# skim0119/gym-softrobot

Hardware: AMD Instinct MI355X
Metric: env_steps_per_sec (higher is better)
Workload: dtype f64

## Files before the change

gym_softrobot_amd/_capi.py:

```python
from __future__ import annotations

import ctypes as C
import os
from pathlib import Path

ABI_VERSION = 17

FEAT_GRAVITY = 1 << 0
FEAT_POINT_FORCE_NODE0_X = 1 << 1
FEAT_PENDULUM_BC = 1 << 2
FEAT_ANALYTICAL_DAMPER = 1 << 3
FEAT_FIXED_BC = 1 << 4
FEAT_TIP_FORCE = 1 << 5
FEAT_MOVING_BASE_BC = 1 << 6
FEAT_LAPLACE_FILTER = 1 << 7
FEAT_PLANE_CONTACT_ANISO = 1 << 8
FEAT_REST_KAPPA_ACTION = 1 << 9
FEAT_OCTO_HEAD = 1 << 10
FEAT_SPLINE_MUSCLE_TORQUES = 1 << 11
FEAT_SUCKER_CONSTRAINT = 1 << 12
FEAT_COOMM_MUSCLES = 1 << 13
MAX_SUCKERS = 4
MAX_MUSCLES = 4
MUSCLE_LONGITUDINAL = 0
# ... 957 lines not shown
    "softrod_bank_info": (C.c_int, [_VP, C.POINTER(C.c_int32), C.POINTER(C.c_uint64), _VP]),
    "softrod_camera_default": (C.c_int, [C.POINTER(SoftrodConfig), C.POINTER(SoftrodCamera)]),
    "softrod_camera_check": (C.c_int, [C.POINTER(SoftrodCamera)]),
    "softrod_render": (C.c_int, [_VP, C.POINTER(SoftrodCamera), _VP, _VP, _VP]),
    "softrod_rod_clearance": (C.c_int, [_VP, C.c_int, _VP, _VP]),
    "softrod_set_rod_shape": (C.c_int, [_VP, _VP, _VP, _VP, _VP, _VP, _VP]),
    "softrod_set_reset_shapes": (C.c_int, [_VP, C.c_int, _VP, _VP, _VP, _VP, C.c_uint64, _VP]),
    "softrod_apply_reset_shapes": (C.c_int, [_VP, _VP, _VP]),
    "softrod_reset_shapes_view": (C.c_int, [_VP, C.POINTER(C.c_void_p), C.POINTER(C.c_void_p)]),
    "softrod_reset_shape_index": (C.c_uint32, [C.c_uint64, C.c_uint32, C.c_uint32, C.c_uint32]),
    "softrod_substeps": (C.c_int, [_VP, _VP, C.c_int, _VP]),
    "softrod_state_view_get": (C.c_int, [_VP, C.POINTER(SoftrodStateView)]),
    "softrod_set_timing": (C.c_int, [_VP, C.c_int]),
    "softrod_kernel_times_ms": (C.c_int, [_VP, _VP, C.c_int, C.POINTER(C.c_int)]),
    "softrod_last_kernel_ms": (C.c_int, [_VP, C.POINTER(C.c_float)]),
    "softrod_kernel_tier": (C.c_char_p, [_VP]),
    "softrod_last_error": (C.c_char_p, [_VP]),
    "softrod_destroy": (C.c_int, [_VP]),
}

EXPORTED_SYMBOLS = tuple(_EXPORTS)

_lib = None


def library_path() -> Path:
    env = os.environ.get("SOFTROD_HIP_LIB")
    if env:
        return Path(env)
    return Path(__file__).resolve().parent / "csrc" / "libsoftrod_hip.so"
# ... 52 lines not shown
```

gym_softrobot_amd/backend.py:

```python
from __future__ import annotations

import ctypes as C
from typing import Dict, Optional, Tuple

import numpy as np
import torch

from . import _capi
from ._capi import LANE_STRIDE, SoftrodConfig, SoftrodStateView, check, load_library
from .diagnostics import (JointLoads, MuscleLoads, RodClearance, RodDynamics, RodStrains, joint_loads_views,
                          muscle_loads_views, rod_clearance_views, rod_dynamics_views, rod_strains_views)


class _DevArray:

    def __init__(self, ptr: int, shape, typestr: str, owner):
        self._owner = owner
        self.__cuda_array_interface__ = {
            "shape": tuple(shape),
            "typestr": typestr,
            "data": (int(ptr), False),
            "version": 2,
            "strides": None,
        }
# ... 478 lines not shown
    def set_timing(self, n_launches: int) -> None:
        check(self._lib.softrod_set_timing(self._h, int(n_launches)), self._h)

    def kernel_times_ms(self) -> np.ndarray:
        cap = 1 << 16
        out = np.zeros(cap, np.float32)
        cnt = C.c_int()
        check(self._lib.softrod_kernel_times_ms(self._h, out.ctypes.data, cap, C.byref(cnt)), self._h)
        return out[: cnt.value].copy()

    def last_kernel_ms(self) -> float:
        ms = C.c_float()
        check(self._lib.softrod_last_kernel_ms(self._h, C.byref(ms)), self._h)
        return float(ms.value)

    def prev_action_rows(self) -> torch.Tensor:
        if getattr(self, "_prev_rows", None) is None:
            self._prev_rows = self.state()["prev_action"]
            if not self.is_octo and not self.is_mocto:
                self._prev_rows = self._prev_rows[:, : self.action_dim]
        return self._prev_rows

    def state(self) -> Dict[str, torch.Tensor]:
        v = SoftrodStateView()
        check(self._lib.softrod_state_view_get(self._h, C.byref(v)), self._h)
        n, s = self.n_envs, int(v.lane_stride)

        def view(ptr, comps):
            return torch.as_tensor(_DevArray(ptr, (comps, n, s), "<f8", self), device=self.device)

# ... 152 lines not shown
```

gym_softrobot_amd/csrc/softrod_capi.hip:

```cpp
#include <hip/hip_runtime.h>
#include <hip/hip_ext.h>

#include <cmath>
#include <cstdio>
#include <cstdlib>
#include <cstring>
#include <new>
#include <string>
#include <vector>

#include "softrod_kernels.hpp"
#include "softrod_dynamics_readout.hpp"
#include "softrod_copy_envs.hpp"
#include "softrod_state_bank.hpp"
#include "softrod_shape.hpp"
#include "softrod_reset_shapes.hpp"

using namespace softrod;

template <class Row>
struct EnvTable {
    Row* dev = nullptr;
    Row* host = nullptr;
    hipEvent_t ev = nullptr;
// ... 48 lines not shown
    RodParams* d_params = nullptr;
    StatePtrs* d_state = nullptr;
    double* d_time_tab = nullptr;
    double* d_mat = nullptr;
    double* d_render_radius = nullptr;
    double* d_mtab = nullptr;
    bool muscles_set = false;
    unsigned* d_ticket = nullptr;
    bool tapered = false;
    bool was_reset = false;
    bool basis_set = false;
    double* h_init = nullptr;
    uint8_t* h_mask = nullptr;
    std::vector<hipEvent_t> ev_start, ev_stop;
    int timed = 0;
    hipEvent_t ev_reset = nullptr;
    int q_depth = 0;
    double* d_queue = nullptr;
    double* h_queue = nullptr;
    int* d_consumed = nullptr;
    int* d_produced = nullptr;
    int* d_underflow = nullptr;
    uint8_t* d_flags = nullptr;
    int* h_produced = nullptr;
    std::vector<int> seen_consumed;
    std::vector<int2> pending;
    double* h_stage = nullptr;
    int2* h_where = nullptr;
    double* d_stage = nullptr;
    int2* d_where = nullptr;
// ... 233 lines not shown
    return SOFTROD_OK;
}

int launch_autoreset_same_step(softrod_handle* h, float* obs, double* aux, int pack, hipStream_t st) {
    const dim3 grid((unsigned)h->cfg.n_envs), block(kLanes * h->nw);
    if (restarts_as_body(h))
        hipLaunchKernelGGL(softrod_octo_autoreset_same_step_kernel, grid, block, 0, st, h->P, h->S, obs, pack, h->d_final_obs,
                           h->d_final_time);
    else
        hipLaunchKernelGGL(by_epl(h, softrod_autoreset_same_step_kernel<1>, softrod_autoreset_same_step_kernel<2>), grid, block,
                           0, st, h->P, h->S, obs, aux, pack, h->d_final_obs, h->d_final_time, h->d_final_aux);
    SR_HIP(h, hipGetLastError());
    return SOFTROD_OK;
}

int launch_reset_shapes(softrod_handle* h, int mode, const uint8_t* mask, float* obs, const uint8_t* term, const uint8_t* trunc,
                        double* aux, int pack, hipStream_t st) {
    const int N = h->cfg.n_envs;
    ResetShapesPick pick{};
    pick.index = h->d_rs_index; pick.episode = h->d_rs_episode; pick.picked = h->d_rs_picked;
    pick.seed = h->rs_seed; pick.count = h->rs_count; pick.mode = mode; pick.mask = mask;
    pick.terminated = pack ? nullptr : term; pick.truncated = pack ? nullptr : trunc;
    pick.packed = (mode == kPickFinished && pack) ? obs : nullptr;
    pick.od = softrod_config_obs_dim(&h->cfg);
    hipLaunchKernelGGL(softrod_reset_shapes_pick_kernel, dim3((unsigned)((N + kPickThreads - 1) / kPickThreads)), dim3(kPickThreads),
                       0, st, h->P, h->S, pick);
    const RodLayout y = rod_layout(h);
    const RodShapeArgs args{h->d_rs_field[0], h->d_rs_field[1], h->d_rs_field[2], h->d_rs_field[3], h->d_rs_picked, h->d_rs_index};
    hipLaunchKernelGGL(by_epl(h, softrod_rod_shape_kernel<1>, softrod_rod_shape_kernel<2>), dim3((unsigned)(N * y.rods)),
                       dim3(kLanes), 0, st, h->P, h->S, y.rods, y.lane_stride, y.arm_stride, args);
// ... 3 lines not shown
                               h->d_rs_picked, obs, pack);
        else
            hipLaunchKernelGGL(by_epl(h, softrod_observe_kernel<1>, softrod_observe_kernel<2>), dim3((unsigned)N), dim3(kLanes), 0,
                               st, h->P, h->S, h->d_rs_picked, nullptr, obs, aux, pack);
    }
    SR_HIP(h, hipGetLastError());
    return SOFTROD_OK;
}

enum : unsigned { kOptMuscles = SOFTROD_FEAT_COOMM_MUSCLES, kOptEarlyTerm = kFeatEarlyTerm, kOptEnvMaterial = kFeatEnvMaterial,
                  kOptEnvContact = kFeatEnvContact, kOptCompiledFor = kOptEarlyTerm | kOptEnvMaterial | kOptEnvContact };
constexpr int kAny = -1, kMoctoEnvs = -2;
constexpr unsigned kAnyFeatures = kRuntimeFeatures;
using StepKernel = void (*)(RodParams, StatePtrs, const float*, float*, double*, uint8_t*, uint8_t*, double*, int, int, int);
using OctoKernel = void (*)(RodParams, StatePtrs, const float*, float*, double*, uint8_t*, uint8_t*, int, int, int);
using WindowKernel = void (*)(RodParams, StatePtrs, const float*, int, int);

struct StepRow {
    unsigned feats;
    int env;
    int math, epl;
    int taper, zup;
    int nw_min, nw_max;
    bool windowed;
    unsigned needs, honours;
    StepKernel step; OctoKernel octo; WindowKernel window;
    int epb, waves;
    const char* label;
};

constexpr StepRow compiled_row(unsigned F, int env, int epl, int taper, int nw_min, int nw_max, const char* label) {
// ... 198 lines not shown
        if (!mask || mask[i]) build(values + W * i, T.host[i]);
    SR_HIP(h, hipMemcpyAsync(T.dev, T.host, N * sizeof(Row), hipMemcpyHostToDevice, st));
    SR_HIP(h, hipEventRecord(T.ev, st));
    return SOFTROD_OK;
}

template <class K, class... A>
void launch_stamped(K kernel, const dim3& grid, const dim3& block, hipStream_t st, hipEvent_t t0, hipEvent_t t1, A... args) {
    if (t0 || t1) hipExtLaunchKernelGGL(kernel, grid, block, 0, st, t0, t1, 0, args...);
    else hipLaunchKernelGGL(kernel, grid, block, 0, st, args...);
}

int launch_step(softrod_handle* h, const float* actions, float* obs, double* reward,
                uint8_t* term, uint8_t* trunc, double* aux, int n_sub, int epilogue, int pack,
                hipStream_t st) {
    if (h->q_depth > 0 && epilogue && !h->same_step) {
        if (const int rc = launch_autoreset(h, obs, reward, term, trunc, aux, pack, st)) return rc;
        if (h->rs_count > 0)
            if (const int rc = launch_reset_shapes(h, kPickSkipped, nullptr, obs, term, trunc, aux, pack, st)) return rc;
    }
    if ((h->cfg.features & SOFTROD_FEAT_COOMM_MUSCLES) && h->cfg.math_mode == SOFTROD_MATH_FAST) {
        const bool push = h->cfg.env_kind == SOFTROD_ENV_ARM_PUSH || is_pull(h) || is_mocto(h);
        if (is_mocto(h) && (!h->tapered || !h->muscles_set || (h->cfg.env_kind == SOFTROD_ENV_ARM_TWO && !h->basis_set)))
            return fail(h, SOFTROD_EINVAL, "the muscle octopus needs softrod_set_radius_profile and softrod_set_muscle_layers "
                                           "(and SOFTROD_ENV_ARM_TWO softrod_set_action_basis) before it steps");
        if (push && !h->tapered)
            return fail(h, SOFTROD_EINVAL, "SOFTROD_ENV_ARM_PUSH (SOFTROD_MATH_FAST): call softrod_set_radius_profile first "
                                           "(the reference's arm is tapered, arm_push_env.py:160-179)");
        if (!push && h->tapered)
            return fail(h, SOFTROD_EINVAL, "a tapered muscle rod outside SOFTROD_ENV_ARM_PUSH runs under SOFTROD_MATH_LIBM only");
    }
    const StepChoice c = select_step(h, epilogue);
    if (!c.row) return fail(h, SOFTROD_EINVAL, c.why);
    const StepChoice after = c.row->windowed ? select_step(h, 0) : StepChoice{nullptr, nullptr};
    if (c.row->windowed && !after.row) return fail(h, SOFTROD_EINVAL, after.why);
    auto launch = [&](const StepRow& r, int n, int epi, hipEvent_t t0, hipEvent_t t1) {
        const dim3 grid((unsigned)((h->cfg.n_envs + r.epb - 1) / r.epb)), block(kLanes * (r.waves ? r.waves : h->nw));
        if (r.window) launch_stamped(r.window, grid, block, st, t0, t1, h->P, h->S, actions, n, h->window_refresh);
        else if (r.octo) launch_stamped(r.octo, grid, block, st, t0, t1, h->P, h->S, actions, obs, reward, term, trunc, n, epi, pack);
        else launch_stamped(r.step, grid, block, st, t0, t1, h->P, h->S, actions, obs, reward, term, trunc, aux, n, epi, pack);
    };
    const bool timing = h->timed < (int)h->ev_start.size();
    const hipEvent_t t0 = timing ? h->ev_start[h->timed] : nullptr, t1 = timing ? h->ev_stop[h->timed] : nullptr;
    const bool mocto = c.row->env == kMoctoEnvs;
    const bool action_first = mocto && epilogue && actions, epilogue_last = mocto && epilogue;
    const dim3 grid((unsigned)h->cfg.n_envs), block(kLanes * h->nw);
    if (action_first)
        launch_stamped(softrod_mocto_action_kernel, grid, block, st, t0, nullptr, h->P, h->S, actions, n_sub);
    launch(*c.row, n_sub, epilogue, action_first ? nullptr : t0, (after.row || epilogue_last) ? nullptr : t1);
    if (after.row) launch(*after.row, 0, 1, nullptr, epilogue_last ? nullptr : t1);
    if (epilogue_last)
        launch_stamped(softrod_mocto_epilogue_kernel, grid, block, st, nullptr, t1, h->P, h->S, obs, reward, term, trunc, 1, pack);
    SR_HIP(h, hipGetLastError());
    if (timing) ++h->timed;
    if (h->q_depth > 0 && epilogue && h->same_step) {
        if (const int rc = launch_autoreset_same_step(h, obs, aux, pack, st)) return rc;
        if (h->rs_count > 0)
            if (const int rc = launch_reset_shapes(h, kPickFinished, nullptr, obs, term, trunc, aux, pack, st)) return rc;
    }
    return SOFTROD_OK;
}

int upload_and_reset(softrod_handle* h, hipStream_t st, bool use_mask) {
    const size_t N = (size_t)h->cfg.n_envs;
    SR_HIP(h, hipMemcpyAsync(h->d_init, h->h_init, N * h->init_stride * sizeof(double), hipMemcpyHostToDevice, st));
    if (use_mask)
        SR_HIP(h, hipMemcpyAsync(h->d_mask, h->h_mask, N, hipMemcpyHostToDevice, st));
    ResetArgs A{h->d_init, use_mask ? h->d_mask : nullptr};
    if (is_octo(h)) {
        OctoResetArgs OA{h->d_init, h->d_init + N * (size_t)h->cfg.n_arm * 18, use_mask ? h->d_mask : nullptr};
        hipLaunchKernelGGL(softrod_octo_reset_kernel, dim3((unsigned)N), dim3(kLanes * h->nw), 0, st, h->P, h->S, OA);
    } else
        hipLaunchKernelGGL(by_epl(h, softrod_reset_kernel<1>, softrod_reset_kernel<2>), dim3((unsigned)N), dim3(kLanes), 0, st,
// ... 1227 lines not shown
        return fail(h, SOFTROD_EINVAL, "null argument");
    if (const int rc = step_preconditions(h)) return rc;
    SR_ON_DEVICE(h);
    return launch_step(h, actions, obs, reward, terminated, truncated, aux, h->cfg.n_substeps, 1, 0,
                       (hipStream_t)stream);
}

int softrod_step_packed(softrod_handle* h, const float* actions, float* packed, double* aux, void* stream) {
    if (!h || !actions || !packed) return fail(h, SOFTROD_EINVAL, "null argument");
    if (const int rc = step_preconditions(h)) return rc;
    SR_ON_DEVICE(h);
    return launch_step(h, actions, packed, nullptr, nullptr, nullptr, aux, h->cfg.n_substeps, 1, 1,
                       (hipStream_t)stream);
}

namespace {
struct PeerTable { float* p[SOFTROD_MAX_PEERS]; };
__global__ void __launch_bounds__(256) softrod_scatter_rows_kernel(const float* __restrict__ packed, PeerTable peers,
                                                                   int n_peers, size_t n_words, size_t offset,
                                                                   long long tag_word, unsigned tag,
                                                                   unsigned* __restrict__ ticket) {
    const size_t i = (size_t)blockIdx.x * blockDim.x + threadIdx.x;
    if (i < n_words) {
        const float v = packed[i];
        for (int q = 0; q < n_peers; ++q)
            __hip_atomic_store(&peers.p[q][offset + i], v, __ATOMIC_RELAXED, __HIP_MEMORY_SCOPE_SYSTEM);
    }
    if (tag_word < 0) return;
    asm volatile("s_waitcnt vmcnt(0)" ::: "memory");
    __syncthreads();
// ... 591 lines not shown
```

gym_softrobot_amd/csrc/softrod_fast.hpp:

```cpp
#pragma once

namespace softrod {

__device__ __forceinline__ bool wave_any(bool p) { return __builtin_amdgcn_ballot_w64(p) != 0ull; }
__device__ __forceinline__ bool wave_any_of(unsigned long long lanes, bool p) {
    return (__builtin_amdgcn_ballot_w64(p) & lanes) != 0ull;
}

__device__ __forceinline__ double horner(double g, double y, double c) {
    double d;
    asm("v_fma_f64 %0, %1, %2, %3" : "=v"(d) : "v"(g), "v"(y), "v"(c));
    return d;
}
__device__ __forceinline__ void fma_over(double& d, double a, double b, double c) {
    asm("v_fma_f64 %0, %1, %2, %3" : "+v"(d) : "v"(a), "v"(b), "v"(c));
}
__device__ __forceinline__ void fma_inplace_u(double& x, double m, double a) {
    asm("v_fma_f64 %0, %1, %0, %2" : "+v"(x) : "s"(m), "v"(a));
}

template <bool LEAN = true, bool ON_CIRCLE = false>
__device__ __forceinline__ void sinc_cosc(double t, double& sc, double& cc) {
    if (!wave_any(t >= 1.0e-3)) {
        if constexpr (LEAN) {
// ... 467 lines not shown
#if SOFTROD_IDLE_LANES_EXEC_MASK
    if (has<F>(P, SOFTROD_FEAT_SPLINE_MUSCLE_TORQUES) || slot_local<F>(P, lane * EPL) <= P.n_elem)
#endif
    {
        constexpr bool kOnCircle = F == kRuntimeFeatures || (F & ~kFeatEnvMaterial) != SOFTROD_FEATURES_SOFTPENDULUM;
        kinematic_n<EPL, kOnCircle>(P.half_dt, C, L);
        ProgressPriority prio(n_sub);
        for (int s = 0; s < n_sub; ++s) {
            dynamic_n<F, EPL, TAPER>(Pk, C, B, lane, L);
            const bool last = (s == n_sub - 1);
            kinematic_n<EPL, kOnCircle>(last ? P.half_dt : P.dt, C, L);
            prio.tick(s);
        }
    }
}
template <unsigned F, int E, int EPL>
__device__ __attribute__((noinline)) void general_step_cold(const RodParams* __restrict__ params,
                                                            const StatePtrs* __restrict__ sp, int rod, int lane,
                                                            const float* __restrict__ actions, int n_sub, int poison) {
    const RodParams P = *params;
    const StatePtrs S = *sp;
    const size_t N = (size_t)P.n_envs;
    LaneN<EPL> L;
    double time;
    if (poison) {
        poison_rod<EPL>(L);
        time = S.time[rod];
    } else {
        load_lane<EPL, F>(S, N, rod, lane, L);
        BcTargets B;
        load_bc(S, N, rod, B);
        EnvAction A;
        set_action_n<F, E, EPL>(P, S, N, rod, lane, actions, A, B, L);
        constrain_rates_n<F, EPL>(P, B, lane, L);
        constrain_values_n<F, EPL>(P, B, lane, L);
        time = S.time[rod];
        if (n_sub > 0) {
            ConstN<EPL> C;
            if constexpr (kEnvMaterial<F>) build_const_m<F, EPL>(P, S.env_mat[rod], lane, A, C);
            else build_const<F, EPL>(P, lane, A, C);
// ... 30 lines not shown
#else
#define SR_PHASE(i) do {} while (0)
#endif

template <unsigned F, int EPL, bool TAPER>
constexpr int fast_kernel_waves() {
    if (EPL > 1) return 1;
    if (F == kRuntimeFeatures) return SOFTROD_RUNTIME_WAVES;
    if (F & (SOFTROD_FEAT_PLANE_CONTACT_ANISO | SOFTROD_FEAT_LAPLACE_FILTER | SOFTROD_FEAT_SPLINE_MUSCLE_TORQUES |
             SOFTROD_FEAT_COOMM_MUSCLES))
        return SOFTROD_CONTACT_WAVES;
    if (TAPER) return SOFTROD_CONTACT_WAVES;
    return (F & ~kFeatEnvMaterial) == SOFTROD_FEATURES_SOFTPENDULUM ? SOFTROD_PLANAR_WAVES : SOFTROD_FAST_WAVES;
}

template <unsigned F, int E, int EPL, bool TAPER = false>
__global__ void __launch_bounds__(kLanes, (fast_kernel_waves<F, EPL, TAPER>()))
softrod_step_fast_kernel(const RodParams P, const StatePtrs S, const float* __restrict__ actions,
                         float* __restrict__ obs, double* __restrict__ reward,
                         uint8_t* __restrict__ terminated, uint8_t* __restrict__ truncated,
                         double* __restrict__ aux, const int n_sub, const int epilogue, const int pack) {
    const int rod = blockIdx.x;
    const int lane = threadIdx.x;
    const size_t N = (size_t)P.n_envs;
    [[maybe_unused]] EnvMaterial M;
    if constexpr (kEnvMaterial<F>) M = S.env_mat[rod];
    [[maybe_unused]] EnvContact CT;
    if constexpr (kEnvContact<F>) CT = S.env_contact[rod];
    if (epilogue && S.skip && S.skip[rod]) {
        if (lane == 0) S.skip[rod] = 0;
        if (lane == 0 && early_term_on<F>(P)) S.aux[rod] = 0.0;
        return;
    }

    __builtin_amdgcn_s_setprio(3);
    SR_PHASE(0);
    constexpr bool kPlanarKernel = (F & ~kFeatEnvMaterial) == SOFTROD_FEATURES_SOFTPENDULUM;
    LaneN<EPL> L;
    load_lane<EPL, F, !kPlanarKernel>(S, N, rod, lane, L);
    SR_PHASE(1);
    if (has<F>(P, SOFTROD_FEAT_LAPLACE_FILTER)) sanitize_unused_rates<EPL>(P, lane, L);
    if (has<F>(P, SOFTROD_FEAT_PLANE_CONTACT_ANISO)) sanitize_unused_slots<EPL>(P, lane, L);
    BcTargets B;
    load_bc(S, N, rod, B);
    load_suckers<F>(P, S, N, rod, B);
    EnvAction A;
    set_action_n<F, E, EPL>(P, S, N, rod, lane, actions, A, B, L);
    if (epilogue) push_store_prev_com<F, E, EPL>(P, S, N, rod, lane, L, n_sub);
    if (has<F>(P, SOFTROD_FEAT_SPLINE_MUSCLE_TORQUES)) muscle_load<EPL>(P, S, rod, actions != nullptr, A, L);
    {
        BcTargets B0 = B;
        if (has<F>(P, SOFTROD_FEAT_MOVING_BASE_BC)) {
            B0.vel[0] = __shfl(L.v[0][0], 0); B0.vel[1] = __shfl(L.v[0][1], 0); B0.vel[2] = __shfl(L.v[0][2], 0);
        }
        constrain_rates_n<F, EPL>(P, B0, lane, L);
        constrain_values_n<F, EPL>(P, B, lane, L);
    }
    double time = S.time[rod];
    ConstN<EPL> C;
    if constexpr (kEnvMaterial<F>) build_const_m<F, EPL, TAPER>(P, M, lane, A, C, S.mat);
    else build_const_m<F, EPL, TAPER>(P, P, lane, A, C, S.mat);
    if constexpr (kEnvContact<F>) C.ct = CT;
    if constexpr (kMusclesCompiled<F>) build_muscle_const<F, EPL, true>(P, S, N, rod, lane, A, C);
    RodParams Pk = P;
    if (!has<F>(P, SOFTROD_FEAT_ANALYTICAL_DAMPER)) Pk.damp_t = 1.0;

    bool blown_up = false;
    if (n_sub > 0 && epilogue && rod_has_nan<EPL>(P, lane, L)) {
        blown_up = true;
        if constexpr (!kPlanarKernel) {
            poison_rod<EPL>(L);
            time = clock_after(P, S, time, n_sub);
        }
    }
    if constexpr (kPlanarKernel) {
        PlanarN<EPL> Z;
        if (n_sub > 0 && !blown_up && planar_from_lane<EPL>(P, B, lane, L, Z)) {
            PlanarC<EPL> K;
            planar_build_const<EPL, kEnvMaterial<F>>(Pk, C, lane, K);
            const double ta = P.time_two_half_adds ? P.half_dt : P.dt;
            const double tb = P.time_two_half_adds ? P.half_dt : 0.0;
            int tk = -1;
            if (S.time_tab && n_sub == P.tab_n_sub) {
                const double kf = rint(time * P.inv_step_time);
                const int k = (kf >= 0.0 && kf < (double)(P.tab_len - 1)) ? (int)kf : -1;
                tk = (k >= 0 && S.time_tab[k] == time) ? k : -1;
            }
            const double step_dt = EPL > 1 ? opaque_v(P.dt) : P.dt;
            SR_PHASE(2);
#if SOFTROD_PLANAR_EXEC_MASK
            if (lane * EPL <= P.n_elem) {
#endif
// ... 24 lines not shown
#endif
            if (__builtin_amdgcn_readfirstlane(tk) >= 0) time = S.time_tab[tk + 1];
            else
                for (int s = 0; s < n_sub; ++s) time = (time + ta) + tb;
            SR_PHASE(3);
            planar_store<EPL>(S, N, rod, lane, Z, !SOFTROD_PLANAR_EXEC_MASK || lane * EPL <= P.n_elem);
#pragma unroll
            for (int s = 0; s < EPL; ++s) {
#pragma unroll
                for (int c = 0; c < 3; ++c) { L.x[s][c] = 0.0; L.v[s][c] = 0.0; L.w[s][c] = 0.0; L.t[s][c] = 0.0; }
#pragma unroll
                for (int c = 0; c < 9; ++c) L.Q[s][c] = 0.0;
            }
            planar_to_lane<EPL>(Z, L);
        } else {
            general_step_cold<F, E, EPL>(S.params, S.self, rod, lane, actions, n_sub, blown_up);
            __builtin_amdgcn_fence(__ATOMIC_ACQUIRE, "wavefront");
            load_lane<EPL, F>(S, N, rod, opaque_lane(lane), L);
            time = S.time[rod];
        }
    } else {
        if (n_sub > 0 && !blown_up) {
            general_substeps<F, EPL, TAPER>(P, Pk, C, B, lane, L, n_sub);
            time = clock_after(P, S, time, n_sub);
        }
        store_lane<EPL, F>(S, N, rod, lane, L);
    }
    if (has<F>(P, SOFTROD_FEAT_SPLINE_MUSCLE_TORQUES)) muscle_store<EPL>(P, S, rod, lane, L);
    if (env_of<E>(P) == SOFTROD_ENV_SOFT_ARM && lane == 0)
        S.ctrl[(size_t)0 * N + rod] += (double)n_sub;
    if (lane == 0) S.time[rod] = time;
// ... 9 lines not shown
```

gym_softrobot_amd/csrc/softrod_kernels.hpp:

```cpp
#pragma once
#include <hip/hip_runtime.h>
#include <stdint.h>

#include "../../include/softrod.h"

namespace softrod {

constexpr int kLanes = 64;

constexpr unsigned kRuntimeFeatures = 0xFFFFFFFFu;
constexpr unsigned kFeaturesTaperedSuckerArm = SOFTROD_FEAT_ANALYTICAL_DAMPER | SOFTROD_FEAT_SUCKER_CONSTRAINT;
constexpr unsigned kFeatPlaneZup = 1u << 30;
constexpr unsigned kFeatEarlyTerm = 1u << 29;
constexpr unsigned kFeatEnvMaterial = 1u << 28;
template <unsigned F>
constexpr bool kEnvMaterial = F != kRuntimeFeatures && (F & kFeatEnvMaterial) != 0;
constexpr unsigned kFeatEnvContact = 1u << 27;
template <unsigned F>
constexpr bool kEnvContact = F != kRuntimeFeatures && (F & kFeatEnvContact) != 0;
constexpr int kRuntimeEnv = -1;
constexpr unsigned kFeaturesMuscleRod = SOFTROD_FEAT_FIXED_BC | SOFTROD_FEAT_ANALYTICAL_DAMPER | SOFTROD_FEAT_COOMM_MUSCLES;
template <unsigned F>
constexpr bool kMusclesCompiled = F != kRuntimeFeatures && (F & SOFTROD_FEAT_COOMM_MUSCLES) != 0;

// ... 1587 lines not shown
        sucker_rates_n<kRuntimeFeatures, 1>(P, B, lane, L);
    }
    if (P.features & SOFTROD_FEAT_ANALYTICAL_DAMPER) {
        L.v[0][0] *= M.damp_t; L.v[0][1] *= M.damp_t; L.v[0][2] *= M.damp_t;
        L.w[0][0] *= pow(M.damp_r[0], e);
        L.w[0][1] *= pow(M.damp_r[1], e);
        L.w[0][2] *= pow(M.damp_r[2], e);
    }
    if (P.features & SOFTROD_FEAT_LAPLACE_FILTER) laplace_filter_rates_n<1>(P, lane, L);
    if (P.damp_before_constrain) {
        constrain_rates_n<kRuntimeFeatures, 1>(P, B, lane, L);
        sucker_rates_n<kRuntimeFeatures, 1>(P, B, lane, L);
    }
}

#ifndef SOFTROD_LIBM_WAVES
#define SOFTROD_LIBM_WAVES 1
#endif
template <bool ET>
__global__ void __launch_bounds__(kLanes, SOFTROD_LIBM_WAVES)
softrod_step_libm_kernel(const RodParams P, const StatePtrs S, const float* __restrict__ actions,
                         float* __restrict__ obs, double* __restrict__ reward,
                         uint8_t* __restrict__ terminated, uint8_t* __restrict__ truncated,
                         double* __restrict__ aux, const int n_sub, const int epilogue, const int pack) {
    const int rod = blockIdx.x;
    const int lane = threadIdx.x;
    const size_t N = (size_t)P.n_envs;
    if (epilogue && S.skip && S.skip[rod]) {
        if (lane == 0) S.skip[rod] = 0;
        if (ET && lane == 0) S.aux[rod] = 0.0;
        return;
    }

    LaneN<1> L;
    load_lane<1, kRuntimeFeatures>(S, N, rod, lane, L);
    BcTargets B;
    load_bc(S, N, rod, B);
    load_suckers<kRuntimeFeatures>(P, S, N, rod, B);
    EnvAction A;
    set_action_n<kRuntimeFeatures, kRuntimeEnv, 1>(P, S, N, rod, lane, actions, A, B, L);
    if (epilogue) push_store_prev_com<kRuntimeFeatures, kRuntimeEnv, 1>(P, S, N, rod, lane, L, n_sub);
    ConstN<1> C;
    const EnvMaterial E = env_material_rt(P, S, rod);
// ... 60 lines not shown
        double a[EPL], o[EPL];
#pragma unroll
        for (int s = 0; s < EPL; ++s) a[s] = x[s][c];
        shift_next<EPL>(a, o);
#pragma unroll
        for (int s = 0; s < EPL; ++s) t[s][c] = o[s] - x[s][c];
    }
#pragma unroll
    for (int s = 0; s < EPL; ++s) {
        const double len = sqrt(t[s][0] * t[s][0] + t[s][1] * t[s][1] + t[s][2] * t[s][2]) + P.eps_length;
#pragma unroll
        for (int c = 0; c < 3; ++c) t[s][c] /= len;
    }
}

__device__ __forceinline__ const double* staged_record(const StatePtrs& S, size_t N, int env, int k) {
    if (k >= S.q_produced[env]) {
        if (threadIdx.x == 0) atomicAdd(S.q_underflow, 1);
        return nullptr;
    }
    return S.queue + ((size_t)(k % S.q_depth) * N + env) * (size_t)S.q_record;
}

template <int EPL>
__global__ void __launch_bounds__(kLanes)
softrod_observe_kernel(const RodParams P, const StatePtrs S, const uint8_t* __restrict__ picked,
                       const float* __restrict__ prev_action, float* __restrict__ obs, double* __restrict__ aux,
                       const int pack) {
    const int rod = blockIdx.x;
    if (picked && !picked[rod]) return;
    const int lane = threadIdx.x;
    const size_t N = (size_t)P.n_envs;
    LaneN<EPL> L;
    load_lane<EPL, kRuntimeFeatures>(S, N, rod, lane, L);
    const int adim = (P.env_kind == SOFTROD_ENV_SOFTPENDULUM3D) ? 2
                   : (P.env_kind == SOFTROD_ENV_ARM_SINGLE) ? 7 : (P.env_kind == SOFTROD_ENV_SOFT_ARM) ? 0
// ... 77 lines not shown
    LaneN<EPL> L;
    reset_rod<EPL>(P, S, (size_t)P.n_envs, rod, threadIdx.x, A.init + (size_t)rod * 18, L);
}

__global__ void __launch_bounds__(kLanes)
softrod_queue_scatter_kernel(double* __restrict__ queue, const double* __restrict__ staged,
                             const int2* __restrict__ where, const int n_envs, const int record) {
    const int m = blockIdx.x;
    const int2 w = where[m];
    double* dst = queue + ((size_t)w.y * (size_t)n_envs + (size_t)w.x) * (size_t)record;
    const double* src = staged + (size_t)m * (size_t)record;
    for (int i = threadIdx.x; i < record; i += kLanes) dst[i] = src[i];
}

template <int EPL>
__global__ void __launch_bounds__(kLanes)
softrod_autoreset_kernel(const RodParams P, const StatePtrs S, float* __restrict__ obs,
                         double* __restrict__ reward, uint8_t* __restrict__ terminated,
                         uint8_t* __restrict__ truncated, double* __restrict__ aux, const int pack) {
    const int rod = blockIdx.x;
    const int lane = threadIdx.x;
    if (!S.needs_reset[rod]) return;
    const size_t N = (size_t)P.n_envs;
    const int k = S.q_consumed[rod];
    const double* in = staged_record(S, N, rod, k);
    if (!in) return;
    LaneN<EPL> L;
    reset_rod<EPL>(P, S, N, rod, lane, in, L);
    float pa[7];
#pragma unroll
    for (int i = 0; i < 7; ++i) pa[i] = S.prev_action[7 * (size_t)rod + i];
    float* o = observe_rod<EPL>(P, S, N, rod, lane, L, pa, obs, pack, aux);
    if (lane == 0) {
        emit_scalars(o, env_obs_dim(P), pack, rod, 0.0, false, false, reward, terminated, truncated, S.needs_reset);
        S.skip[rod] = 1;
        S.q_consumed[rod] = k + 1;
    }
}

}

#include "softrod_fast.hpp"
#include "softrod_octo.hpp"
#include "softrod_window.hpp"
#include "softrod_literal.hpp"
#include "softrod_readout.hpp"
#include "softrod_reaction.hpp"
#include "softrod_strains.hpp"
#include "softrod_muscle_readout.hpp"
#include "softrod_joint_readout.hpp"
#include "softrod_render.hpp"
#include "softrod_clearance.hpp"
// ... 2 lines not shown
```

gym_softrobot_amd/csrc/softrod_window.hpp:

```cpp
#pragma once

namespace softrod {

constexpr int kWindowRho = 4;

template <unsigned F>
__device__ __forceinline__ void window_load(const StatePtrs& S, size_t N, int rod, int g, LaneN<1>& L) {
    constexpr size_t W = 2 * kLanes;
    const size_t m = (size_t)rod * W + (size_t)g;
#pragma unroll
    for (int c = 0; c < 3; ++c) {
        L.x[0][c] = S.pos[c * N * W + m];
        L.v[0][c] = S.vel[c * N * W + m];
        L.w[0][c] = S.omg[c * N * W + m];
        L.t[0][c] = S.tan[c * N * W + m];
        L.kap[0][c] = S.kap[c * N * W + m];
        L.rk[0][c] = S.rkap[c * N * W + m];
    }
#pragma unroll
    for (int c = 0; c < 9; ++c) L.Q[0][c] = S.dir[c * N * W + m];
}

__device__ __forceinline__ void window_store(const StatePtrs& S, size_t N, int rod, int g, const LaneN<1>& L) {
    constexpr size_t W = 2 * kLanes;
// ... 1 lines not shown
#pragma unroll
    for (int c = 0; c < 3; ++c) {
        S.pos[c * N * W + m] = L.x[0][c];
        S.vel[c * N * W + m] = L.v[0][c];
        S.omg[c * N * W + m] = L.w[0][c];
        S.tan[c * N * W + m] = L.t[0][c];
        S.kap[c * N * W + m] = L.kap[0][c];
    }
#pragma unroll
    for (int c = 0; c < 9; ++c) S.dir[c * N * W + m] = L.Q[0][c];
}

template <unsigned F, int RPB = 1>
__global__ void __launch_bounds__(2 * kLanes * RPB, SOFTROD_CONTACT_WAVES)
softrod_step_window_kernel(const RodParams P, const StatePtrs S, const float* __restrict__ actions,
                           const int n_sub, const int refresh) {
    static_assert(RPB == 1 || RPB == 4, "one rod per workgroup, or four with partner waves on one SIMD");
    constexpr int kFields = 18;
    constexpr int kHalo = (RPB == 1) ? kLanes : 32;
    constexpr int kBuf = (RPB == 1) ? 1 : 2;
    __shared__ double ex_[RPB][kBuf][2][kFields][kHalo];
    __shared__ int flag_[RPB][2];
    __shared__ int sany_[RPB];

    const int wib = threadIdx.x >> 6;
    const int es = (RPB == 1) ? 0 : (wib & (RPB - 1));
    const int wave = (RPB == 1) ? wib : (wib / RPB);
    const int lane = threadIdx.x & 63;
    const int tid = wave * kLanes + lane;
    const bool active = (RPB == 1) || ((int)blockIdx.x * RPB + es < P.n_envs);
    const int rod = active ? (int)blockIdx.x * RPB + es : P.n_envs - 1;
    auto& ex = ex_[es];
    const size_t N = (size_t)P.n_envs;
    const int n = P.n_elem;
    bool live = active && !(S.skip && S.skip[rod]);
    if constexpr (RPB == 1) { if (!live) return; }
    const int off = wave ? (n + 1 - kLanes) : 0;
    const int g = off + lane;
    const int split = (n + 1) / 2;
    const bool owned = wave ? (g >= split) : (g < split);
    const int gi = (wave == 0 && lane == kLanes - 1) ? n : g;
    if constexpr (RPB > 1) {
        if (tid < 2) flag_[es][tid] = 0;
        if (tid == 0) sany_[es] = 0;
    }

    LaneN<1> L;
    window_load<F>(S, N, rod, g, L);
    if (actions) {
        double rk0 = 0.0;
        if (g < n - 1) {
// ... 64 lines not shown
    {
        bool bad = false;
#pragma unroll
        for (int c = 0; c < 3; ++c)
            bad = bad || (owned && (isnan(L.x[0][c]) || isnan(L.v[0][c]) || (g < n && isnan(L.w[0][c]))));
#pragma unroll
        for (int c = 0; c < 9; ++c) bad = bad || (owned && g < n && isnan(L.Q[0][c]));
        if constexpr (RPB == 1) dead = __syncthreads_or(bad ? 1 : 0) != 0;
        else {
            __syncthreads();
            if (__any(bad) && lane == 0) atomicOr(&sany_[es], 1);
            __syncthreads();
            dead = sany_[es] != 0;
        }
    }
    if (!live) return;
    if (dead) {
        poison_rod<1>(L);
    } else if (n_sub > 0) {
        kinematic_n<1>(P.half_dt, C, L);
        int since = 0;
        for (int s = 0; s < n_sub; ++s) {
            if constexpr (RPB > 1) {
                if (since == 0) __builtin_amdgcn_s_setprio(2);
                else if (since == 1) __builtin_amdgcn_s_setprio(1);
                else __builtin_amdgcn_s_setprio(0);
            }
            dynamic_n<F, 1>(Pk, C, B, gi, L);
            const bool last = (s == n_sub - 1);
            kinematic_n<1>(last ? P.half_dt : P.dt, C, L);
            if (++since == refresh) { exchange(); since = 0; }
// ... 13 lines not shown
```

include/softrod.h:

```cpp
#ifndef SOFTROD_H
#define SOFTROD_H

#include <stddef.h>
#include <stdint.h>

#ifdef __cplusplus
extern "C" {
#endif

#define SOFTROD_ABI_VERSION 17

#define SOFTROD_OK 0
#define SOFTROD_EINVAL (-1)
#define SOFTROD_ENOMEM (-2)
#define SOFTROD_EHIP (-3)
#define SOFTROD_ENODEV (-4)

enum softrod_feature {
    SOFTROD_FEAT_GRAVITY = 1u << 0,
    SOFTROD_FEAT_POINT_FORCE_NODE0_X = 1u << 1,
    SOFTROD_FEAT_PENDULUM_BC = 1u << 2,
    SOFTROD_FEAT_ANALYTICAL_DAMPER = 1u << 3,
    SOFTROD_FEAT_FIXED_BC = 1u << 4,
    SOFTROD_FEAT_TIP_FORCE = 1u << 5,
// ... 281 lines not shown

int softrod_set_reset_shapes(softrod_handle* h, int count, const double* kappa, const double* sigma, const double* velocity,
                             const double* omega, uint64_t seed, void* stream);
int softrod_apply_reset_shapes(softrod_handle* h, const uint8_t* mask, void* stream);
int softrod_reset_shapes_view(softrod_handle* h, int32_t** index, int32_t** episode);
uint32_t softrod_reset_shape_index(uint64_t seed, uint32_t env, uint32_t episode, uint32_t count);

int softrod_substeps(softrod_handle* h, const float* actions, int n, void* stream);

int softrod_state_view_get(softrod_handle* h, softrod_state_view* out);

int softrod_set_timing(softrod_handle* h, int n_launches);
int softrod_kernel_times_ms(softrod_handle* h, float* out_ms, int cap, int* count);
int softrod_last_kernel_ms(softrod_handle* h, float* ms);

const char* softrod_kernel_tier(softrod_handle* h);

const char* softrod_last_error(softrod_handle* h);
int softrod_destroy(softrod_handle* h);
int softrod_abi_version(void);
const char* softrod_source_hash(void);

#ifdef __cplusplus
}
#endif
#endif
```

Baseline: 14.20 million.

## Fold next-step auto-reset into the step kernel to drop a dispatch

Result: faster. 14.36 million (median of 6 runs) (+1.2%).

```diff
diff --git a/gym_softrobot_amd/_capi.py b/gym_softrobot_amd/_capi.py
--- a/gym_softrobot_amd/_capi.py
+++ b/gym_softrobot_amd/_capi.py
@@ -995,6 +995,7 @@
     "softrod_set_timing": (C.c_int, [_VP, C.c_int]),
     "softrod_kernel_times_ms": (C.c_int, [_VP, _VP, C.c_int, C.POINTER(C.c_int)]),
     "softrod_last_kernel_ms": (C.c_int, [_VP, C.POINTER(C.c_float)]),
+    "softrod_last_step_dispatches": (C.c_int, [_VP, C.POINTER(C.c_int)]),
     "softrod_kernel_tier": (C.c_char_p, [_VP]),
     "softrod_last_error": (C.c_char_p, [_VP]),
     "softrod_destroy": (C.c_int, [_VP]),
diff --git a/gym_softrobot_amd/backend.py b/gym_softrobot_amd/backend.py
--- a/gym_softrobot_amd/backend.py
+++ b/gym_softrobot_amd/backend.py
@@ -516,6 +516,11 @@
         check(self._lib.softrod_last_kernel_ms(self._h, C.byref(ms)), self._h)
         return float(ms.value)
 
+    def last_step_dispatches(self) -> int:
+        n = C.c_int()
+        check(self._lib.softrod_last_step_dispatches(self._h, C.byref(n)), self._h)
+        return int(n.value)
+
     def prev_action_rows(self) -> torch.Tensor:
         if getattr(self, "_prev_rows", None) is None:
             self._prev_rows = self.state()["prev_action"]
diff --git a/gym_softrobot_amd/csrc/softrod_capi.hip b/gym_softrobot_amd/csrc/softrod_capi.hip
--- a/gym_softrobot_amd/csrc/softrod_capi.hip
+++ b/gym_softrobot_amd/csrc/softrod_capi.hip
@@ -86,6 +86,7 @@
     uint8_t* h_mask = nullptr;
     std::vector<hipEvent_t> ev_start, ev_stop;
     int timed = 0;
+    int step_dispatches = 0;
     hipEvent_t ev_reset = nullptr;
     int q_depth = 0;
     double* d_queue = nullptr;
@@ -349,6 +350,7 @@
     return SOFTROD_OK;
 }
 
+constexpr int kResetShapesDispatches = 3;
 int launch_reset_shapes(softrod_handle* h, int mode, const uint8_t* mask, float* obs, const uint8_t* term, const uint8_t* trunc,
                         double* aux, int pack, hipStream_t st) {
     const int N = h->cfg.n_envs;
@@ -382,7 +384,7 @@
 constexpr unsigned kAnyFeatures = kRuntimeFeatures;
 using StepKernel = void (*)(RodParams, StatePtrs, const float*, float*, double*, uint8_t*, uint8_t*, double*, int, int, int);
 using OctoKernel = void (*)(RodParams, StatePtrs, const float*, float*, double*, uint8_t*, uint8_t*, int, int, int);
-using WindowKernel = void (*)(RodParams, StatePtrs, const float*, int, int);
+using WindowKernel = void (*)(RodParams, StatePtrs, const float*, int, int, StepOut, int);
 
 struct StepRow {
     unsigned feats;
@@ -611,10 +613,16 @@
 int launch_step(softrod_handle* h, const float* actions, float* obs, double* reward,
                 uint8_t* term, uint8_t* trunc, double* aux, int n_sub, int epilogue, int pack,
                 hipStream_t st) {
-    if (h->q_depth > 0 && epilogue && !h->same_step) {
+    h->step_dispatches = 0;
+    const bool next_step = h->q_depth > 0 && epilogue && !h->same_step;
+    const bool fused = next_step && !restarts_as_body(h) && h->rs_count == 0 && (h->epl == 1 || h->window_refresh > 0);
+    if (next_step && !fused) {
         if (const int rc = launch_autoreset(h, obs, reward, term, trunc, aux, pack, st)) return rc;
-        if (h->rs_count > 0)
+        ++h->step_dispatches;
+        if (h->rs_count > 0) {
             if (const int rc = launch_reset_shapes(h, kPickSkipped, nullptr, obs, term, trunc, aux, pack, st)) return rc;
+            h->step_dispatches += kResetShapesDispatches;
+        }
     }
     if ((h->cfg.features & SOFTROD_FEAT_COOMM_MUSCLES) && h->cfg.math_mode == SOFTROD_MATH_FAST) {
         const bool push = h->cfg.env_kind == SOFTROD_ENV_ARM_PUSH || is_pull(h) || is_mocto(h);
@@ -631,29 +639,44 @@
     if (!c.row) return fail(h, SOFTROD_EINVAL, c.why);
     const StepChoice after = c.row->windowed ? select_step(h, 0) : StepChoice{nullptr, nullptr};
     if (c.row->windowed && !after.row) return fail(h, SOFTROD_EINVAL, after.why);
-    auto launch = [&](const StepRow& r, int n, int epi, hipEvent_t t0, hipEvent_t t1) {
+    if (fused && (c.row->octo || (!c.row->window && c.row->epl != 1)))
+        return fail(h, SOFTROD_EINVAL, "device auto-reset: the handle's step kernel does not restart finished envs");
+    auto launch = [&](const StepRow& r, int n, int epi, bool first, hipEvent_t t0, hipEvent_t t1) {
         const dim3 grid((unsigned)((h->cfg.n_envs + r.epb - 1) / r.epb)), block(kLanes * (r.waves ? r.waves : h->nw));
-        if (r.window) launch_stamped(r.window, grid, block, st, t0, t1, h->P, h->S, actions, n, h->window_refresh);
+        const int restart = fused && first;
+        if (r.window)
+            launch_stamped(r.window, grid, block, st, t0, t1, h->P, h->S, actions, n, h->window_refresh,
+                           StepOut{obs, reward, term, trunc, aux, pack}, restart);
         else if (r.octo) launch_stamped(r.octo, grid, block, st, t0, t1, h->P, h->S, actions, obs, reward, term, trunc, n, epi, pack);
-        else launch_stamped(r.step, grid, block, st, t0, t1, h->P, h->S, actions, obs, reward, term, trunc, aux, n, epi, pack);
+        else
+            launch_stamped(r.step, grid, block, st, t0, t1, h->P, h->S, actions, obs, reward, term, trunc, aux, n,
+                           epi | (restart ? kEpilogueRestart : 0), pack);
+        ++h->step_dispatches;
     };
     const bool timing = h->timed < (int)h->ev_start.size();
     const hipEvent_t t0 = timing ? h->ev_start[h->timed] : nullptr, t1 = timing ? h->ev_stop[h->timed] : nullptr;
     const bool mocto = c.row->env == kMoctoEnvs;
     const bool action_first = mocto && epilogue && actions, epilogue_last = mocto && epilogue;
     const dim3 grid((unsigned)h->cfg.n_envs), block(kLanes * h->nw);
-    if (action_first)
+    if (action_first) {
         launch_stamped(softrod_mocto_action_kernel, grid, block, st, t0, nullptr, h->P, h->S, actions, n_sub);
-    launch(*c.row, n_sub, epilogue, action_first ? nullptr : t0, (after.row || epilogue_last) ? nullptr : t1);
-    if (after.row) launch(*after.row, 0, 1, nullptr, epilogue_last ? nullptr : t1);
-    if (epilogue_last)
+        ++h->step_dispatches;
+    }
+    launch(*c.row, n_sub, epilogue, true, action_first ? nullptr : t0, (after.row || epilogue_last) ? nullptr : t1);
+    if (after.row) launch(*after.row, 0, 1, false, nullptr, epilogue_last ? nullptr : t1);
+    if (epilogue_last) {
         launch_stamped(softrod_mocto_epilogue_kernel, grid, block, st, nullptr, t1, h->P, h->S, obs, reward, term, trunc, 1, pack);
+        ++h->step_dispatches;
+    }
     SR_HIP(h, hipGetLastError());
     if (timing) ++h->timed;
     if (h->q_depth > 0 && epilogue && h->same_step) {
         if (const int rc = launch_autoreset_same_step(h, obs, aux, pack, st)) return rc;
-        if (h->rs_count > 0)
+        ++h->step_dispatches;
+        if (h->rs_count > 0) {
             if (const int rc = launch_reset_shapes(h, kPickFinished, nullptr, obs, term, trunc, aux, pack, st)) return rc;
+            h->step_dispatches += kResetShapesDispatches;
+        }
     }
     return SOFTROD_OK;
 }
@@ -1911,6 +1934,12 @@
                        (hipStream_t)stream);
 }
 
+int softrod_last_step_dispatches(softrod_handle* h, int* out) {
+    if (!h || !out) return fail(h, SOFTROD_EINVAL, "last step dispatches: null argument");
+    *out = h->step_dispatches;
+    return SOFTROD_OK;
+}
+
 namespace {
 struct PeerTable { float* p[SOFTROD_MAX_PEERS]; };
 __global__ void __launch_bounds__(256) softrod_scatter_rows_kernel(const float* __restrict__ packed, PeerTable peers,
diff --git a/gym_softrobot_amd/csrc/softrod_fast.hpp b/gym_softrobot_amd/csrc/softrod_fast.hpp
--- a/gym_softrobot_amd/csrc/softrod_fast.hpp
+++ b/gym_softrobot_amd/csrc/softrod_fast.hpp
@@ -505,16 +505,23 @@
         }
     }
 }
+enum : int { kColdStep = 0, kColdPoison = 1, kColdRestart = 2 };
 template <unsigned F, int E, int EPL>
 __device__ __attribute__((noinline)) void general_step_cold(const RodParams* __restrict__ params,
                                                             const StatePtrs* __restrict__ sp, int rod, int lane,
-                                                            const float* __restrict__ actions, int n_sub, int poison) {
+                                                            const float* __restrict__ actions, int n_sub, int mode,
+                                                            StepOut O) {
     const RodParams P = *params;
     const StatePtrs S = *sp;
     const size_t N = (size_t)P.n_envs;
+    if (mode == kColdRestart) {
+        const int k = S.q_consumed[rod];
+        restart_rod<EPL>(P, S, N, rod, lane, k, staged_at(S, N, rod, k), O, false);
+        return;
+    }
     LaneN<EPL> L;
     double time;
-    if (poison) {
+    if (mode == kColdPoison) {
         poison_rod<EPL>(L);
         time = S.time[rod];
     } else {
@@ -575,6 +582,46 @@
     return (F & ~kFeatEnvMaterial) == SOFTROD_FEATURES_SOFTPENDULUM ? SOFTROD_PLANAR_WAVES : SOFTROD_FAST_WAVES;
 }
 
+template <unsigned F, int E, int EPL, bool TAPER>
+__device__ __forceinline__ void step_prologue(const RodParams& P, const StatePtrs& S, size_t N, int rod, int lane,
+                                              const float* __restrict__ actions, int n_sub, int epilogue,
+                                              const EnvMaterial& M, const EnvContact& CT, LaneN<EPL>& L, BcTargets& B,
+                                              EnvAction& A, ConstN<EPL>& C, double& time, bool& blown_up) {
+    constexpr bool kPlanarKernel = (F & ~kFeatEnvMaterial) == SOFTROD_FEATURES_SOFTPENDULUM;
+    __builtin_amdgcn_s_setprio(3);
+    SR_PHASE(0);
+    load_lane<EPL, F, !kPlanarKernel>(S, N, rod, lane, L);
+    SR_PHASE(1);
+    if (has<F>(P, SOFTROD_FEAT_LAPLACE_FILTER)) sanitize_unused_rates<EPL>(P, lane, L);
+    if (has<F>(P, SOFTROD_FEAT_PLANE_CONTACT_ANISO)) sanitize_unused_slots<EPL>(P, lane, L);
+    load_bc(S, N, rod, B);
+    load_suckers<F>(P, S, N, rod, B);
+    set_action_n<F, E, EPL>(P, S, N, rod, lane, actions, A, B, L);
+    if (epilogue) push_store_prev_com<F, E, EPL>(P, S, N, rod, lane, L, n_sub);
+    if (has<F>(P, SOFTROD_FEAT_SPLINE_MUSCLE_TORQUES)) muscle_load<EPL>(P, S, rod, actions != nullptr, A, L);
+    {
+        BcTargets B0 = B;
+        if (has<F>(P, SOFTROD_FEAT_MOVING_BASE_BC)) {
+            B0.vel[0] = __shfl(L.v[0][0], 0); B0.vel[1] = __shfl(L.v[0][1], 0); B0.vel[2] = __shfl(L.v[0][2], 0);
+        }
+        constrain_rates_n<F, EPL>(P, B0, lane, L);
+        constrain_values_n<F, EPL>(P, B, lane, L);
+    }
+    time = S.time[rod];
+    if constexpr (kEnvMaterial<F>) build_const_m<F, EPL, TAPER>(P, M, lane, A, C, S.mat);
+    else build_const_m<F, EPL, TAPER>(P, P, lane, A, C, S.mat);
+    if constexpr (kEnvContact<F>) C.ct = CT;
+    if constexpr (kMusclesCompiled<F>) build_muscle_const<F, EPL, true>(P, S, N, rod, lane, A, C);
+
+    if (n_sub > 0 && epilogue && rod_has_nan<EPL>(P, lane, L)) {
+        blown_up = true;
+        if constexpr (!kPlanarKernel) {
+            poison_rod<EPL>(L);
+            time = clock_after(P, S, time, n_sub);
+        }
+    }
+}
+
 template <unsigned F, int E, int EPL, bool TAPER = false>
 __global__ void __launch_bounds__(kLanes, (fast_kernel_waves<F, EPL, TAPER>()))
 softrod_step_fast_kernel(const RodParams P, const StatePtrs S, const float* __restrict__ actions,
@@ -588,55 +635,37 @@
     if constexpr (kEnvMaterial<F>) M = S.env_mat[rod];
     [[maybe_unused]] EnvContact CT;
     if constexpr (kEnvContact<F>) CT = S.env_contact[rod];
-    if (epilogue && S.skip && S.skip[rod]) {
+    constexpr bool kPlanarKernel = (F & ~kFeatEnvMaterial) == SOFTROD_FEATURES_SOFTPENDULUM;
+    constexpr bool kRestarts = EPL == 1;
+    bool restart = false;
+    if (kRestarts && (epilogue & kEpilogueRestart)) {
+        restart = restart_due(S, rod, lane == 0);
+        if constexpr (!kPlanarKernel) {
+            if (restart) {
+                restart_next_step_cold<EPL, false>(S.self, rod, lane, StepOut{obs, reward, terminated, truncated, aux, pack});
+                if (lane == 0 && early_term_on<F>(P)) S.aux[rod] = 0.0;
+                return;
+            }
+        }
+    } else if (epilogue && S.skip && S.skip[rod]) {
         if (lane == 0) S.skip[rod] = 0;
         if (lane == 0 && early_term_on<F>(P)) S.aux[rod] = 0.0;
         return;
     }
 
-    __builtin_amdgcn_s_setprio(3);
-    SR_PHASE(0);
-    constexpr bool kPlanarKernel = (F & ~kFeatEnvMaterial) == SOFTROD_FEATURES_SOFTPENDULUM;
     LaneN<EPL> L;
-    load_lane<EPL, F, !kPlanarKernel>(S, N, rod, lane, L);
-    SR_PHASE(1);
-    if (has<F>(P, SOFTROD_FEAT_LAPLACE_FILTER)) sanitize_unused_rates<EPL>(P, lane, L);
-    if (has<F>(P, SOFTROD_FEAT_PLANE_CONTACT_ANISO)) sanitize_unused_slots<EPL>(P, lane, L);
     BcTargets B;
-    load_bc(S, N, rod, B);
-    load_suckers<F>(P, S, N, rod, B);
     EnvAction A;
-    set_action_n<F, E, EPL>(P, S, N, rod, lane, actions, A, B, L);
-    if (epilogue) push_store_prev_com<F, E, EPL>(P, S, N, rod, lane, L, n_sub);
-    if (has<F>(P, SOFTROD_FEAT_SPLINE_MUSCLE_TORQUES)) muscle_load<EPL>(P, S, rod, actions != nullptr, A, L);
-    {
-        BcTargets B0 = B;
-        if (has<F>(P, SOFTROD_FEAT_MOVING_BASE_BC)) {
-            B0.vel[0] = __shfl(L.v[0][0], 0); B0.vel[1] = __shfl(L.v[0][1], 0); B0.vel[2] = __shfl(L.v[0][2], 0);
-        }
-        constrain_rates_n<F, EPL>(P, B0, lane, L);
-        constrain_values_n<F, EPL>(P, B, lane, L);
-    }
-    double time = S.time[rod];
     ConstN<EPL> C;
-    if constexpr (kEnvMaterial<F>) build_const_m<F, EPL, TAPER>(P, M, lane, A, C, S.mat);
-    else build_const_m<F, EPL, TAPER>(P, P, lane, A, C, S.mat);
-    if constexpr (kEnvContact<F>) C.ct = CT;
-    if constexpr (kMusclesCompiled<F>) build_muscle_const<F, EPL, true>(P, S, N, rod, lane, A, C);
+    double time = 0.0;
+    bool blown_up = false;
+    if (!kPlanarKernel || !restart)
+        step_prologue<F, E, EPL, TAPER>(P, S, N, rod, lane, actions, n_sub, epilogue, M, CT, L, B, A, C, time, blown_up);
     RodParams Pk = P;
     if (!has<F>(P, SOFTROD_FEAT_ANALYTICAL_DAMPER)) Pk.damp_t = 1.0;
-
-    bool blown_up = false;
-    if (n_sub > 0 && epilogue && rod_has_nan<EPL>(P, lane, L)) {
-        blown_up = true;
-        if constexpr (!kPlanarKernel) {
-            poison_rod<EPL>(L);
-            time = clock_after(P, S, time, n_sub);
-        }
-    }
     if constexpr (kPlanarKernel) {
         PlanarN<EPL> Z;
-        if (n_sub > 0 && !blown_up && planar_from_lane<EPL>(P, B, lane, L, Z)) {
+        if (!restart && n_sub > 0 && !blown_up && planar_from_lane<EPL>(P, B, lane, L, Z)) {
             PlanarC<EPL> K;
             planar_build_const<EPL, kEnvMaterial<F>>(Pk, C, lane, K);
             const double ta = P.time_two_half_adds ? P.half_dt : P.dt;
@@ -691,7 +720,10 @@
             }
             planar_to_lane<EPL>(Z, L);
         } else {
-            general_step_cold<F, E, EPL>(S.params, S.self, rod, lane, actions, n_sub, blown_up);
+            general_step_cold<F, E, EPL>(S.params, S.self, rod, lane, actions, n_sub,
+                                         restart ? kColdRestart : blown_up ? kColdPoison : kColdStep,
+                                         StepOut{obs, reward, terminated, truncated, aux, pack});
+            if (restart) return;
             __builtin_amdgcn_fence(__ATOMIC_ACQUIRE, "wavefront");
             load_lane<EPL, F>(S, N, rod, opaque_lane(lane), L);
             time = S.time[rod];
diff --git a/gym_softrobot_amd/csrc/softrod_kernels.hpp b/gym_softrobot_amd/csrc/softrod_kernels.hpp
--- a/gym_softrobot_amd/csrc/softrod_kernels.hpp
+++ b/gym_softrobot_amd/csrc/softrod_kernels.hpp
@@ -1625,6 +1625,22 @@
     }
 }
 
+constexpr int kEpilogue = 1, kEpilogueRestart = 2;
+struct StepOut {
+    float* obs; double* reward; uint8_t* terminated; uint8_t* truncated; double* aux; int pack;
+};
+__device__ __forceinline__ bool restart_due(const StatePtrs& S, int rod, bool counter) {
+    if (!S.needs_reset[rod]) return false;
+    if (S.q_consumed[rod] >= S.q_produced[rod]) {
+        if (counter) atomicAdd(S.q_underflow, 1);
+        return false;
+    }
+    return true;
+}
+template <int EPL, bool MARK_SKIP>
+__device__ __attribute__((noinline)) void restart_next_step_cold(const StatePtrs* __restrict__ sp, int rod, int lane,
+                                                                 StepOut O);
+
 #ifndef SOFTROD_LIBM_WAVES
 #define SOFTROD_LIBM_WAVES 1
 #endif
@@ -1637,7 +1653,13 @@
     const int rod = blockIdx.x;
     const int lane = threadIdx.x;
     const size_t N = (size_t)P.n_envs;
-    if (epilogue && S.skip && S.skip[rod]) {
+    if (epilogue & kEpilogueRestart) {
+        if (restart_due(S, rod, lane == 0)) {
+            restart_next_step_cold<1, false>(S.self, rod, lane, StepOut{obs, reward, terminated, truncated, aux, pack});
+            if (ET && lane == 0) S.aux[rod] = 0.0;
+            return;
+        }
+    } else if (epilogue && S.skip && S.skip[rod]) {
         if (lane == 0) S.skip[rod] = 0;
         if (ET && lane == 0) S.aux[rod] = 0.0;
         return;
@@ -1728,12 +1750,15 @@
     }
 }
 
+__device__ __forceinline__ const double* staged_at(const StatePtrs& S, size_t N, int env, int k) {
+    return S.queue + ((size_t)(k % S.q_depth) * N + env) * (size_t)S.q_record;
+}
 __device__ __forceinline__ const double* staged_record(const StatePtrs& S, size_t N, int env, int k) {
     if (k >= S.q_produced[env]) {
         if (threadIdx.x == 0) atomicAdd(S.q_underflow, 1);
         return nullptr;
     }
-    return S.queue + ((size_t)(k % S.q_depth) * N + env) * (size_t)S.q_record;
+    return staged_at(S, N, env, k);
 }
 
 template <int EPL>
@@ -1841,6 +1866,22 @@
 }
 
 template <int EPL>
+__device__ __forceinline__ void restart_rod(const RodParams& P, const StatePtrs& S, size_t N, int rod, int lane, int k,
+                                            const double* __restrict__ in, const StepOut& O, bool mark_skip) {
+    LaneN<EPL> L;
+    reset_rod<EPL>(P, S, N, rod, lane, in, L);
+    float pa[7];
+#pragma unroll
+    for (int i = 0; i < 7; ++i) pa[i] = S.prev_action[7 * (size_t)rod + i];
+    float* o = observe_rod<EPL>(P, S, N, rod, lane, L, pa, O.obs, O.pack, O.aux);
+    if (lane == 0) {
+        emit_scalars(o, env_obs_dim(P), O.pack, rod, 0.0, false, false, O.reward, O.terminated, O.truncated, S.needs_reset);
+        if (mark_skip) S.skip[rod] = 1;
+        S.q_consumed[rod] = k + 1;
+    }
+}
+
+template <int EPL>
 __global__ void __launch_bounds__(kLanes)
 softrod_autoreset_kernel(const RodParams P, const StatePtrs S, float* __restrict__ obs,
                          double* __restrict__ reward, uint8_t* __restrict__ terminated,
@@ -1852,17 +1893,17 @@
     const int k = S.q_consumed[rod];
     const double* in = staged_record(S, N, rod, k);
     if (!in) return;
-    LaneN<EPL> L;
-    reset_rod<EPL>(P, S, N, rod, lane, in, L);
-    float pa[7];
-#pragma unroll
-    for (int i = 0; i < 7; ++i) pa[i] = S.prev_action[7 * (size_t)rod + i];
-    float* o = observe_rod<EPL>(P, S, N, rod, lane, L, pa, obs, pack, aux);
-    if (lane == 0) {
-        emit_scalars(o, env_obs_dim(P), pack, rod, 0.0, false, false, reward, terminated, truncated, S.needs_reset);
-        S.skip[rod] = 1;
-        S.q_consumed[rod] = k + 1;
-    }
+    restart_rod<EPL>(P, S, N, rod, lane, k, in, StepOut{obs, reward, terminated, truncated, aux, pack}, true);
+}
+
+template <int EPL, bool MARK_SKIP>
+__device__ __attribute__((noinline)) void restart_next_step_cold(const StatePtrs* __restrict__ sp, int rod, int lane,
+                                                                 StepOut O) {
+    const StatePtrs S = *sp;
+    const RodParams P = *S.params;
+    const size_t N = (size_t)P.n_envs;
+    const int k = S.q_consumed[rod];
+    restart_rod<EPL>(P, S, N, rod, lane, k, staged_at(S, N, rod, k), O, MARK_SKIP);
 }
 
 }
diff --git a/gym_softrobot_amd/csrc/softrod_window.hpp b/gym_softrobot_amd/csrc/softrod_window.hpp
--- a/gym_softrobot_amd/csrc/softrod_window.hpp
+++ b/gym_softrobot_amd/csrc/softrod_window.hpp
@@ -39,7 +39,7 @@
 template <unsigned F, int RPB = 1>
 __global__ void __launch_bounds__(2 * kLanes * RPB, SOFTROD_CONTACT_WAVES)
 softrod_step_window_kernel(const RodParams P, const StatePtrs S, const float* __restrict__ actions,
-                           const int n_sub, const int refresh) {
+                           const int n_sub, const int refresh, const StepOut O, const int restart) {
     static_assert(RPB == 1 || RPB == 4, "one rod per workgroup, or four with partner waves on one SIMD");
     constexpr int kFields = 18;
     constexpr int kHalo = (RPB == 1) ? kLanes : 32;
@@ -58,8 +58,15 @@
     auto& ex = ex_[es];
     const size_t N = (size_t)P.n_envs;
     const int n = P.n_elem;
-    bool live = active && !(S.skip && S.skip[rod]);
-    if constexpr (RPB == 1) { if (!live) return; }
+    const bool fresh = restart && active && restart_due(S, rod, tid == 0);
+    bool live = active && !fresh && !(!restart && S.skip && S.skip[rod]);
+    if constexpr (RPB == 1) {
+        if (restart) __syncthreads();
+        if (!live) {
+            if (fresh && wave == 0) restart_next_step_cold<2, true>(S.self, rod, lane, O);
+            return;
+        }
+    }
     const int off = wave ? (n + 1 - kLanes) : 0;
     const int g = off + lane;
     const int split = (n + 1) / 2;
@@ -154,7 +161,12 @@
             dead = sany_[es] != 0;
         }
     }
-    if (!live) return;
+    if constexpr (RPB > 1) {
+        if (!live) {
+            if (fresh && wave == 0) restart_next_step_cold<2, true>(S.self, rod, lane, O);
+            return;
+        }
+    }
     if (dead) {
         poison_rod<1>(L);
     } else if (n_sub > 0) {
diff --git a/include/softrod.h b/include/softrod.h
--- a/include/softrod.h
+++ b/include/softrod.h
@@ -319,6 +319,8 @@
 int softrod_kernel_times_ms(softrod_handle* h, float* out_ms, int cap, int* count);
 int softrod_last_kernel_ms(softrod_handle* h, float* ms);
 
+int softrod_last_step_dispatches(softrod_handle* h, int* out);
+
 const char* softrod_kernel_tier(softrod_handle* h);
 
 const char* softrod_last_error(softrod_handle* h);
```
